# xrsrke/pipegoose

Measured on AMD Instinct MI355X. Metric: tokens/sec, higher is better.
Workload: dtype bf16; 1 GPU; model=bloom-560m, global_batch=8, seq_len=2048, parallelism=tp1pp1dp1

## Files before the change

pipegoose_amd/ops/csrc/attention.hip:

```cpp
#include <torch/extension.h>
#include <ATen/cuda/CUDAContext.h>

#include "common.h"

namespace {

using bf16 = __hip_bfloat16;
using frag_ab = __attribute__((ext_vector_type(8))) __bf16;
using frag_cd = __attribute__((ext_vector_type(4))) float;

__device__ __forceinline__ frag_cd MFMA_16x16x32(frag_ab a, frag_ab b, frag_cd c) {
    return __builtin_amdgcn_mfma_f32_16x16x32_bf16(a, b, c, 0, 0, 0);
}

constexpr int BLOCK_M = 64;
constexpr int BLOCK_N = 64;
constexpr int NWAVES = 4;
constexpr int PAD = 8;
constexpr float NEG_INF = -1e30f;


template <int D, int MT, int WAVES = NWAVES>
__global__ __launch_bounds__(WAVES * WAVE_SIZE)
void attn_fwd_kernel(const bf16* __restrict__ q, const bf16* __restrict__ k,
// ... 137 lines not shown
#pragma unroll
                for (int r = 0; r < 4; ++r) accO[mt][s][r] *= rescale[r];
            }

#pragma unroll
            for (int ns = 0; ns < 4; ++ns) {
#pragma unroll
                for (int r = 0; r < 4; ++r) {
                    float pv = __expf(s_tile[ns][r] - m_run[mt][r]);
                    s_tile[ns][r] = pv;
                    p_lds[wave][(mt * 16 + 4 * lgrp + r) * VSTRIDE + ns * 16 + lcol] =
                        (bf16)pv;
                }
            }
#pragma unroll
            for (int r = 0; r < 4; ++r) {
                float ls = s_tile[0][r] + s_tile[1][r] + s_tile[2][r] + s_tile[3][r];
#pragma unroll
                for (int off = 1; off < 16; off <<= 1) {
                    ls += __shfl_xor(ls, off, WAVE_SIZE);
                }
                l_run[mt][r] += ls;
            }
        }
        __builtin_amdgcn_s_waitcnt(0);

#pragma unroll
        for (int mt = 0; mt < MT; ++mt) {
#pragma unroll
            for (int kc = 0; kc < 2; ++kc) {
                frag_ab aP = *reinterpret_cast<const frag_ab*>(
                    &p_lds[wave][(mt * 16 + lcol) * VSTRIDE + kc * 32 + 8 * lgrp]);
                __builtin_amdgcn_s_setprio(1);
#pragma unroll
                for (int ds = 0; ds < DSUB; ++ds) {
                    frag_ab bV = *reinterpret_cast<const frag_ab*>(
                        &vt_lds[(ds * 16 + lcol) * VSTRIDE + kc * 32 + 8 * lgrp]);
                    accO[mt][ds] = MFMA_16x16x32(aP, bV, accO[mt][ds]);
                }
                __builtin_amdgcn_s_setprio(0);
            }
        }
    }

#pragma unroll
    for (int mt = 0; mt < MT; ++mt) {
#pragma unroll
        for (int r = 0; r < 4; ++r) {
            const int iq = qrow0 + mt * 16 + 4 * lgrp + r;
            const float inv_l = 1.0f / l_run[mt][r];
            bf16* orow = op + (int64_t)iq * os;
#pragma unroll
            for (int ds = 0; ds < DSUB; ++ds) {
                orow[ds * 16 + lcol] = (bf16)(accO[mt][ds][r] * inv_l);
            }
            if (lcol == 0) {
                lse[bh_off + iq] = m_run[mt][r] + __logf(l_run[mt][r]);
            }
        }
    }
}

__global__ void mfma_probe_kernel(const bf16* __restrict__ A,
                                  const bf16* __restrict__ Bt,
                                  float* __restrict__ C) {
    const int lane = threadIdx.x;
    const int lgrp = lane >> 4, lcol = lane & 15;
    frag_ab a = *reinterpret_cast<const frag_ab*>(A + lcol * 32 + 8 * lgrp);
    frag_ab b = *reinterpret_cast<const frag_ab*>(Bt + lcol * 32 + 8 * lgrp);
    frag_cd c = MFMA_16x16x32(a, b, frag_cd{0.f, 0.f, 0.f, 0.f});
#pragma unroll
    for (int r = 0; r < 4; ++r) {
        C[(4 * lgrp + r) * 16 + lcol] = c[r];
    }
}

}

__device__ __forceinline__ float u2f(unsigned u) { return __uint_as_float(u); }

namespace {

using f32x16 = __attribute__((ext_vector_type(16))) float;
using bf16x4 = __attribute__((ext_vector_type(4))) __bf16;
using lds_bf16x4_p = __attribute__((address_space(3))) bf16x4*;

__device__ __forceinline__ f32x16 MFMA_32x32x16(frag_ab a, frag_ab b, f32x16 c) {
    return __builtin_amdgcn_mfma_f32_32x32x16_bf16(a, b, c, 0, 0, 0);
}

__device__ __forceinline__ int swz128(int row, int elem_col) {
    return row * 128 + ((((elem_col) << 1) ^ ((row & 15) << 4)) >> 1);
}

__device__ __forceinline__ int swz64(int row, int elem_col) {
    return row * 64 + ((((elem_col) << 1) ^ ((row & 7) << 4)) >> 1);
}

template <int RS>
__device__ __forceinline__ int swz_rm(int row, int elem_col) {
    return RS == 64 ? swz64(row, elem_col) : swz128(row, elem_col);
}

template <int D> __device__ __forceinline__ int bwd_rm(int row, int col) {
    return D == 64 ? row * 72 + col : swz128(row, col);
}
template <int D> __device__ __forceinline__ int bwd_tr(int row, int col) {
    return D == 64 ? row * 40 + col : swz64(row, col);
}

template <int D>
__device__ __forceinline__ void pkt_rc(int p, int& row, int& col) {
    constexpr int DLOG = (D / 16 == 8) ? 3 : 2;
    const int rw = (p >> 1) & 3;
    const int dd = (p >> 3) & (D / 16 - 1);
    row = (p >> (3 + DLOG)) * 4 + rw;
    col = dd * 16 + (p & 1) * 8;
}

template <int D, int WAVES>
__global__ __launch_bounds__(WAVES * WAVE_SIZE)
void attn_fwd_v2_kernel(const bf16* __restrict__ q, const bf16* __restrict__ k,
                        const bf16* __restrict__ v,
                        const float* __restrict__ slopes, float scale,
                        bf16* __restrict__ o, float* __restrict__ lse,
                        int B, int H, int S, int kv_off, int kv_group,
                        int64_t qb, int64_t qh, int64_t qs,
                        int64_t kb, int64_t kh, int64_t ks,
                        int64_t vb, int64_t vh, int64_t vs,
                        int64_t ob, int64_t oh, int64_t os) {
    constexpr int KVB = 64;
    constexpr int NT = WAVES * WAVE_SIZE;
    constexpr int ROWS = WAVES * 32;
    constexpr int DCH = D / 16;
    constexpr int DSUB = D / 32;
    constexpr int NPK = KVB * (D / 8);
    constexpr int NPV = KVB * (D / 8);
    constexpr int KPL = (NPK + NT - 1) / NT;
    constexpr int VPL = (NPV + NT - 1) / NT;
    constexpr int VST = (D / 16) * 64;

    __shared__ __attribute__((aligned(16))) bf16 k_lds[2][KVB * 128];
    __shared__ __attribute__((aligned(16))) bf16 vs_lds[2][KVB * D];

    int qblock = blockIdx.x, h = blockIdx.y, b = blockIdx.z;
    {
        const int ngrp = gridDim.y * gridDim.z;
        if ((ngrp & 7) == 0) {
            const int flat = blockIdx.x +
                gridDim.x * (blockIdx.y + gridDim.y * blockIdx.z);
            qblock = flat / ngrp;
            const int g = flat % ngrp;
            h = g % gridDim.y;
            b = g / gridDim.y;
        }
    }
    const int tid = threadIdx.x;
    const int wave = tid / WAVE_SIZE;
    const int lane = tid % WAVE_SIZE;
    const int l31 = lane & 31;
    const int hi = lane >> 5;

    const int64_t bh_off = ((int64_t)b * H + h) * S;
    const int hk = h / kv_group;
    const bf16* qp = q + b * qb + h * qh;
    const bf16* kp = k + b * kb + hk * kh;
// ... 55 lines not shown
    auto stage_write = [&](int buf) {
#pragma unroll
        for (int i = 0; i < KPL; ++i) {
            const int p = tid + i * NT;
            if (p < NPK) {
                const int row = p / (D / 8);
                const int col = (p % (D / 8)) * 8;
                *reinterpret_cast<frag_ab*>(&k_lds[buf][swz128(row, col)]) =
                    kreg[i];
            }
        }
#pragma unroll
        for (int i = 0; i < VPL; ++i) {
            const int p = tid + i * NT;
            if (p < NPV) {
                int row, col;
                pkt_rc<D>(p, row, col);
                const int idx = (row >> 2) * VST + (col >> 4) * 64 +
                                (row & 3) * 16 + (col & 15);
                *reinterpret_cast<frag_ab*>(&vs_lds[buf][idx]) = vreg[i];
            }
        }
    };

    if (nkv > 0) {
        stage_load(0);
        stage_write(0);
    }
    __syncthreads();

    for (int nb = 0; nb < nkv; ++nb) {
        const int cur = nb & 1;
        const int kvrow0 = nb * KVB;
        const bool last = (nb + 1 == nkv);
        if (!last) stage_load(nb + 1);

        const bool active = full_vis || (kvrow0 + kv_off <= qr0 + 31);

        f32x16 st[2];
        frag_ab pfrag[4];
        if (active) {
#pragma unroll
            for (int ns = 0; ns < 2; ++ns) {
#pragma unroll
                for (int r = 0; r < 16; ++r) st[ns][r] = 0.f;
            }
#pragma unroll
            for (int ns = 0; ns < 2; ++ns) {
                __builtin_amdgcn_s_setprio(1);
#pragma unroll
                for (int c = 0; c < DCH; ++c) {
                    frag_ab aK = *reinterpret_cast<const frag_ab*>(
                        &k_lds[cur][swz128(ns * 32 + l31, c * 16 + 8 * hi)]);
                    st[ns] = MFMA_32x32x16(aK, bQ[c], st[ns]);
                }
                __builtin_amdgcn_s_setprio(0);
            }

            float mr[32];
#pragma unroll
            for (int ns = 0; ns < 2; ++ns) {
#pragma unroll
                for (int r = 0; r < 16; ++r) {
                    const int jk = kvrow0 + ns * 32 + (r & 3) + 8 * (r >> 2) +
                                   4 * hi + kv_off;
                    float x = st[ns][r] * scale2 + slope2 * (float)(jk - iq);
                    x = (jk <= iq) ? x : NEG_INF;
                    st[ns][r] = x;
                    mr[ns * 16 + r] = x;
                }
            }
#pragma unroll
            for (int w = 16; w > 0; w >>= 1) {
#pragma unroll
                for (int i = 0; i < w; ++i) mr[i] = fmaxf(mr[i], mr[i + w]);
            }
            float mx = mr[0];
            {
                auto sw = __builtin_amdgcn_permlane32_swap(
                    __float_as_uint(mx), __float_as_uint(mx), false, false);
                mx = fmaxf(u2f(sw[0]), u2f(sw[1]));
            }
            const float m_new = fmaxf(m_run, mx);
            const float alpha = exp2f(m_run - m_new);
            m_run = m_new;
            l_run *= alpha;
#pragma unroll
            for (int dsb = 0; dsb < DSUB; ++dsb) {
#pragma unroll
                for (int r = 0; r < 16; ++r) accO[dsb][r] *= alpha;
            }
            float sr[32];
#pragma unroll
            for (int ns = 0; ns < 2; ++ns) {
#pragma unroll
                for (int r = 0; r < 16; ++r) {
                    const float pv = exp2f(st[ns][r] - m_new);
                    st[ns][r] = pv;
                    sr[ns * 16 + r] = pv;
                }
            }
#pragma unroll
            for (int w = 16; w > 0; w >>= 1) {
#pragma unroll
                for (int i = 0; i < w; ++i) sr[i] += sr[i + w];
            }
            float ls = sr[0];
            {
                auto sw = __builtin_amdgcn_permlane32_swap(
                    __float_as_uint(ls), __float_as_uint(ls), false, false);
                ls = u2f(sw[0]) + u2f(sw[1]);
            }
            l_run += ls;

#pragma unroll
            for (int ns = 0; ns < 2; ++ns) {
#pragma unroll
                for (int hf = 0; hf < 2; ++hf) {
                    union { __bf16 h2[2]; uint32_t u; } wa, wb, wc, wd;
                    wa.h2[0] = (__bf16)st[ns][8 * hf + 0];
                    wa.h2[1] = (__bf16)st[ns][8 * hf + 1];
                    wc.h2[0] = (__bf16)st[ns][8 * hf + 2];
                    wc.h2[1] = (__bf16)st[ns][8 * hf + 3];
                    wb.h2[0] = (__bf16)st[ns][8 * hf + 4];
                    wb.h2[1] = (__bf16)st[ns][8 * hf + 5];
                    wd.h2[0] = (__bf16)st[ns][8 * hf + 6];
                    wd.h2[1] = (__bf16)st[ns][8 * hf + 7];
                    auto s1 = __builtin_amdgcn_permlane32_swap(wa.u, wb.u,
                                                              false, false);
                    auto s2 = __builtin_amdgcn_permlane32_swap(wc.u, wd.u,
                                                              false, false);
                    union { frag_ab f; uint32_t u[4]; } out;
                    out.u[0] = s1[0];
                    out.u[1] = s2[0];
                    out.u[2] = s1[1];
                    out.u[3] = s2[1];
                    pfrag[2 * ns + hf] = out.f;
                }
            }
        }

        if (!last) stage_write(cur ^ 1);

        if (active) {
            const int lq = lane >> 4;
            const int dblk_off = (lq & 1) * 64;
            const int lel = (lane & 15) * 4;
#pragma unroll
            for (int dsb = 0; dsb < DSUB; ++dsb) {
                __builtin_amdgcn_s_setprio(1);
#pragma unroll
                for (int ks2 = 0; ks2 < 4; ++ks2) {
                    const int g0 = 4 * ks2 + 2 * hi;
                    const int base = g0 * VST + (2 * dsb) * 64 + dblk_off + lel;
                    union { frag_ab f; bf16x4 h[2]; } av;
                    av.h[0] = __builtin_amdgcn_ds_read_tr16_b64_v4bf16(
                        (lds_bf16x4_p)&vs_lds[cur][base]);
                    av.h[1] = __builtin_amdgcn_ds_read_tr16_b64_v4bf16(
                        (lds_bf16x4_p)&vs_lds[cur][base + VST]);
                    accO[dsb] = MFMA_32x32x16(av.f, pfrag[ks2], accO[dsb]);
                }
                __builtin_amdgcn_s_setprio(0);
            }
        }
        __syncthreads();
    }

    const float inv_l = (l_run > 0.f) ? 1.0f / l_run : 0.f;
    bf16* orow = op + (int64_t)iq * os;
#pragma unroll
    for (int dsb = 0; dsb < DSUB; ++dsb) {
#pragma unroll
        for (int g = 0; g < 4; ++g) {
            union { __bf16 h4[4]; uint2 u; } w;
#pragma unroll
            for (int r = 0; r < 4; ++r) {
                w.h4[r] = (__bf16)(accO[dsb][4 * g + r] * inv_l);
            }
            *reinterpret_cast<uint2*>(orow + dsb * 32 + 8 * g + 4 * hi) = w.u;
        }
// ... 441 lines not shown
        : min((int64_t)S, (int64_t)qb * QROWS + QROWS - kv_off);
    for (int kv0 = 0; kv0 < kv_end; kv0 += KVR) {
        __syncthreads();
        {
            constexpr int PACKETS = (KVR / 2) * (D / 8);
            for (int p = tid; p < PACKETS; p += NT) {
                const int row = (p / (D / 8)) * 2;
                const int col = (p % (D / 8)) * 8;
                frag_ab pk0 = *reinterpret_cast<const frag_ab*>(
                    kp + (int64_t)(kv0 + row) * ks2 + col);
                frag_ab pk1 = *reinterpret_cast<const frag_ab*>(
                    kp + (int64_t)(kv0 + row + 1) * ks2 + col);
                frag_ab pv0 = *reinterpret_cast<const frag_ab*>(
                    vp + (int64_t)(kv0 + row) * vs2 + col);
                frag_ab pv1 = *reinterpret_cast<const frag_ab*>(
                    vp + (int64_t)(kv0 + row + 1) * vs2 + col);
                *reinterpret_cast<frag_ab*>(&k_lds[bwd_rm<D>(row, col)]) = pk0;
                *reinterpret_cast<frag_ab*>(&k_lds[bwd_rm<D>(row + 1, col)]) = pk1;
                *reinterpret_cast<frag_ab*>(&v_lds[bwd_rm<D>(row, col)]) = pv0;
                *reinterpret_cast<frag_ab*>(&v_lds[bwd_rm<D>(row + 1, col)]) = pv1;
#pragma unroll
                for (int j = 0; j < 8; ++j) {
                    union { __bf16 h[2]; uint32_t u; } a;
                    a.h[0] = pk0[j]; a.h[1] = pk1[j];
                    *reinterpret_cast<uint32_t*>(&kt_lds[bwd_tr<D>(col + j, row)]) = a.u;
                }
            }
        }
        __syncthreads();

#pragma unroll
        for (int ns = 0; ns < KVR / 16; ++ns) {
            frag_cd sacc = frag_cd{0.f, 0.f, 0.f, 0.f};
            frag_cd dpacc = frag_cd{0.f, 0.f, 0.f, 0.f};
#pragma unroll
            for (int c = 0; c < DCH; ++c) {
                frag_ab bK = *reinterpret_cast<const frag_ab*>(
                    &k_lds[bwd_rm<D>(ns * 16 + lcol, c * 32 + 8 * lgrp)]);
                sacc = MFMA_16x16x32(aQ[c], bK, sacc);
                frag_ab bV = *reinterpret_cast<const frag_ab*>(
                    &v_lds[bwd_rm<D>(ns * 16 + lcol, c * 32 + 8 * lgrp)]);
                dpacc = MFMA_16x16x32(aDO[c], bV, dpacc);
            }
#pragma unroll
            for (int r = 0; r < 4; ++r) {
                const int iq = qrow0 + 4 * lgrp + r;
                const int jk = kv0 + ns * 16 + lcol + kv_off;
                float z = sacc[r] * scale2 + slope2 * (float)(jk - iq);
                float p = (jk <= iq) ? exp2f(z - lse_r[r]) : 0.f;
                float ds = p * (dpacc[r] - delta_r[r]) * scale;
                ds_lds[wave][bwd_tr<D>(4 * lgrp + r, ns * 16 + lcol)] = (bf16)ds;
            }
        }
        __builtin_amdgcn_s_waitcnt(0);

#pragma unroll
        for (int kc = 0; kc < KVR / 32; ++kc) {
            frag_ab aDS = *reinterpret_cast<const frag_ab*>(
                &ds_lds[wave][bwd_tr<D>(lcol, kc * 32 + 8 * lgrp)]);
#pragma unroll
            for (int ds = 0; ds < DSUB; ++ds) {
                frag_ab bKT = *reinterpret_cast<const frag_ab*>(
                    &kt_lds[bwd_tr<D>(ds * 16 + lcol, kc * 32 + 8 * lgrp)]);
                accDQ[ds] = MFMA_16x16x32(aDS, bKT, accDQ[ds]);
            }
        }
    }

#pragma unroll
    for (int r = 0; r < 4; ++r) {
        const int iq = qrow0 + 4 * lgrp + r;
        bf16* dqrow = dq + b * wb + h * wh + (int64_t)iq * ws;
#pragma unroll
        for (int ds = 0; ds < DSUB; ++ds) {
            dqrow[ds * 16 + lcol] = (bf16)accDQ[ds][r];
        }
    }
}

}

namespace {

template <int D>
__device__ __forceinline__ int sub_idx(int row, int elem_col) {
    constexpr int DBLK = D / 16;
    const int g = row >> 2;
    const int dblk = (elem_col >> 4) ^ (g & (DBLK - 1));
    return g * (DBLK * 64) + dblk * 64 + (row & 3) * 16 + (elem_col & 15);
}

template <int D>
__device__ __forceinline__ int sub_tile_base(int g, int dblk_log) {
    constexpr int DBLK = D / 16;
    return g * (DBLK * 64) + (dblk_log ^ (g & (DBLK - 1))) * 64;
}

template <int D, int WAVES>
__global__ __launch_bounds__(WAVES * WAVE_SIZE)
void attn_bwd_dq_v2_kernel(const bf16* __restrict__ dout,
                           const bf16* __restrict__ q, const bf16* __restrict__ k,
                           const bf16* __restrict__ v,
                           const float* __restrict__ lse,
                           const float* __restrict__ delta,
                           const float* __restrict__ slopes, float scale,
                           bf16* __restrict__ dq,
                           int B, int H, int S, int kv_off, int kv_group,
                           int64_t gb, int64_t gh, int64_t gs,
                           int64_t qb2, int64_t qh2, int64_t qs2,
                           int64_t kb2, int64_t kh2, int64_t ks2,
                           int64_t vb2, int64_t vh2, int64_t vs2,
                           int64_t wb, int64_t wh, int64_t ws) {
    constexpr int KVB = 64;
    constexpr int NT = WAVES * WAVE_SIZE;
    constexpr int ROWS = WAVES * 32;
    constexpr int DCH = D / 16;
    constexpr int DSUB = D / 32;
    constexpr int VST = (D / 16) * 64;
    constexpr int NPK = KVB * (D / 8);
    constexpr int KPL = (NPK + NT - 1) / NT;
    constexpr int NP = (KVB / 2) * (D / 8);
    constexpr int PPL = (NP + NT - 1) / NT;

    __shared__ __attribute__((aligned(16))) bf16 ks_lds[2][KVB * D];
    __shared__ __attribute__((aligned(16))) bf16 v_lds[2][KVB * 128];

    const int qblock = blockIdx.x;
    const int h = blockIdx.y;
    const int b = blockIdx.z;
    const int tid = threadIdx.x;
    const int wave = tid / WAVE_SIZE;
    const int lane = tid % WAVE_SIZE;
    const int l31 = lane & 31;
    const int hi = lane >> 5;
    const int lq = lane >> 4;

    const int64_t bh_off = ((int64_t)b * H + h) * S;
    const int hk = h / kv_group;
    const bf16* kp = k + b * kb2 + hk * kh2;
    const bf16* vp = v + b * vb2 + hk * vh2;
    const float LOG2E = 1.4426950408889634f;
    const float scale2 = scale * LOG2E;
    const float slope2 = slopes[h] * LOG2E;

    const int qr0 = qblock * ROWS + wave * 32;
    const int iq = qr0 + l31;

    frag_ab bQ[DCH], bDO[DCH];
    {
        const bf16* qrow = q + b * qb2 + h * qh2 + (int64_t)iq * qs2;
        const bf16* dorow = dout + b * gb + h * gh + (int64_t)iq * gs;
#pragma unroll
        for (int c = 0; c < DCH; ++c) {
            bQ[c] = *reinterpret_cast<const frag_ab*>(qrow + c * 16 + 8 * hi);
            bDO[c] = *reinterpret_cast<const frag_ab*>(dorow + c * 16 + 8 * hi);
        }
    }
    const float lse2 = lse[bh_off + iq] * LOG2E;
    const float dlt = delta[bh_off + iq];

    f32x16 accDQ[DSUB];
#pragma unroll
    for (int dsb = 0; dsb < DSUB; ++dsb) {
#pragma unroll
        for (int r = 0; r < 16; ++r) accDQ[dsb][r] = 0.f;
    }

    const bool full_vis = (kv_off <= -S);
    const int kv_end = full_vis ? S
        : min(S, qblock * ROWS + ROWS - kv_off);
    const int nkv = max(0, (kv_end + KVB - 1) / KVB);

    frag_ab kreg[KPL], vreg[PPL][2];
    auto stage_load = [&](int nb) {
        const int kvrow0 = nb * KVB;
#pragma unroll
        for (int i = 0; i < KPL; ++i) {
            const int p = tid + i * NT;
            if (p < NPK) {
                int row, col;
                pkt_rc<D>(p, row, col);
                kreg[i] = *reinterpret_cast<const frag_ab*>(
                    kp + (int64_t)(kvrow0 + row) * ks2 + col);
            }
        }
#pragma unroll
        for (int i = 0; i < PPL; ++i) {
            const int p = tid + i * NT;
            if (p < NP) {
                const int row = (p / (D / 8)) * 2;
                const int col = (p % (D / 8)) * 8;
                vreg[i][0] = *reinterpret_cast<const frag_ab*>(
                    vp + (int64_t)(kvrow0 + row) * vs2 + col);
                vreg[i][1] = *reinterpret_cast<const frag_ab*>(
                    vp + (int64_t)(kvrow0 + row + 1) * vs2 + col);
            }
        }
    };
    auto stage_write = [&](int buf) {
#pragma unroll
        for (int i = 0; i < KPL; ++i) {
            const int p = tid + i * NT;
            if (p < NPK) {
                int row, col;
                pkt_rc<D>(p, row, col);
                *reinterpret_cast<frag_ab*>(
                    &ks_lds[buf][sub_idx<D>(row, col)]) = kreg[i];
            }
        }
#pragma unroll
        for (int i = 0; i < PPL; ++i) {
            const int p = tid + i * NT;
            if (p < NP) {
                const int row = (p / (D / 8)) * 2;
                const int col = (p % (D / 8)) * 8;
#pragma unroll
                for (int rr = 0; rr < 2; ++rr) {
                    *reinterpret_cast<frag_ab*>(
                        &v_lds[buf][swz128(row + rr, col)]) = vreg[i][rr];
                }
            }
        }
    };

    constexpr bool EARLY_LOAD = true;
    if (nkv > 0) {
        stage_load(0);
        stage_write(0);
    }
    __syncthreads();

    for (int nb = 0; nb < nkv; ++nb) {
        const int cur = nb & 1;
        const int kvrow0 = nb * KVB;
        const bool last = (nb + 1 == nkv);
        if (EARLY_LOAD && !last) stage_load(nb + 1);

        const bool active = full_vis || (kvrow0 + kv_off <= qr0 + 31);
        if (active) {
            auto ns_body = [&](int ns) {
                frag_ab dsfrag[2];
                f32x16 st, dp;
#pragma unroll
                for (int r = 0; r < 16; ++r) { st[r] = 0.f; dp[r] = 0.f; }
                __builtin_amdgcn_s_setprio(1);
#pragma unroll
                for (int c = 0; c < DCH; ++c) {
                    frag_ab aK = *reinterpret_cast<const frag_ab*>(
                        &ks_lds[cur][sub_idx<D>(ns * 32 + l31, c * 16 + 8 * hi)]);
                    st = MFMA_32x32x16(aK, bQ[c], st);
                    frag_ab aV = *reinterpret_cast<const frag_ab*>(
                        &v_lds[cur][swz128(ns * 32 + l31, c * 16 + 8 * hi)]);
                    dp = MFMA_32x32x16(aV, bDO[c], dp);
                }
                __builtin_amdgcn_s_setprio(0);
#pragma unroll
                for (int r = 0; r < 16; ++r) {
                    const int jk = kvrow0 + ns * 32 + (r & 3) + 8 * (r >> 2) +
                                   4 * hi + kv_off;
                    const float z2 = st[r] * scale2 +
                                     slope2 * (float)(jk - iq);
                    const float p = (jk <= iq) ? exp2f(z2 - lse2) : 0.f;
                    st[r] = p * (dp[r] - dlt) * scale;
                }
#pragma unroll
                for (int hf = 0; hf < 2; ++hf) {
                    union { __bf16 h2[2]; uint32_t u; } wa, wb2, wc, wd;
                    wa.h2[0] = (__bf16)st[8 * hf + 0];
                    wa.h2[1] = (__bf16)st[8 * hf + 1];
                    wc.h2[0] = (__bf16)st[8 * hf + 2];
                    wc.h2[1] = (__bf16)st[8 * hf + 3];
                    wb2.h2[0] = (__bf16)st[8 * hf + 4];
                    wb2.h2[1] = (__bf16)st[8 * hf + 5];
                    wd.h2[0] = (__bf16)st[8 * hf + 6];
                    wd.h2[1] = (__bf16)st[8 * hf + 7];
                    auto s1 = __builtin_amdgcn_permlane32_swap(wa.u, wb2.u,
                                                              false, false);
                    auto s2 = __builtin_amdgcn_permlane32_swap(wc.u, wd.u,
                                                              false, false);
                    union { frag_ab f; uint32_t u[4]; } out;
                    out.u[0] = s1[0];
                    out.u[1] = s2[0];
                    out.u[2] = s1[1];
                    out.u[3] = s2[1];
                    dsfrag[hf] = out.f;
                }
#pragma unroll
                for (int dsb = 0; dsb < DSUB; ++dsb) {
                    __builtin_amdgcn_s_setprio(1);
#pragma unroll
                    for (int ksq = 0; ksq < 2; ++ksq) {
                        const int g0 = 8 * ns + 4 * ksq + 2 * hi;
                        const int dblk = 2 * dsb + (lq & 1);
                        union { frag_ab f; bf16x4 h[2]; } akt;
                        akt.h[0] = __builtin_amdgcn_ds_read_tr16_b64_v4bf16(
                            (lds_bf16x4_p)&ks_lds[cur][
                                sub_tile_base<D>(g0, dblk) + (lane & 15) * 4]);
                        akt.h[1] = __builtin_amdgcn_ds_read_tr16_b64_v4bf16(
                            (lds_bf16x4_p)&ks_lds[cur][
                                sub_tile_base<D>(g0 + 1, dblk) + (lane & 15) * 4]);
                        accDQ[dsb] = MFMA_32x32x16(akt.f, dsfrag[ksq],
                                                   accDQ[dsb]);
                    }
                    __builtin_amdgcn_s_setprio(0);
                }
            };
            if (D == 128) {
#pragma unroll 1
                for (int ns = 0; ns < 2; ++ns) ns_body(ns);
            } else {
                ns_body(0);
                ns_body(1);
            }
        }
        if (!last) {
            if (!EARLY_LOAD) stage_load(nb + 1);
            stage_write(cur ^ 1);
        }
        __syncthreads();
    }

    bf16* dqrow = dq + b * wb + h * wh + (int64_t)iq * ws;
#pragma unroll
    for (int dsb = 0; dsb < DSUB; ++dsb) {
#pragma unroll
        for (int g = 0; g < 4; ++g) {
            union { __bf16 h4[4]; uint2 u; } w;
#pragma unroll
            for (int r = 0; r < 4; ++r) w.h4[r] = (__bf16)accDQ[dsb][4 * g + r];
            *reinterpret_cast<uint2*>(dqrow + dsb * 32 + 8 * g + 4 * hi) = w.u;
        }
    }
}

template <int D, int WAVES, bool DO_DK, bool DO_DV, int DKPART = -1>
__global__ __launch_bounds__(WAVES * WAVE_SIZE)
void attn_bwd_dkdv_v2_kernel(const bf16* __restrict__ dout,
                             const bf16* __restrict__ q, const bf16* __restrict__ k,
                             const bf16* __restrict__ v,
                             const float* __restrict__ lse,
                             const float* __restrict__ delta,
                             const float* __restrict__ slopes, float scale,
                             bf16* __restrict__ dk, bf16* __restrict__ dv,
                             int B, int H, int S, int kv_off, int kv_group,
                             int64_t gb, int64_t gh, int64_t gs,
                             int64_t qb2, int64_t qh2, int64_t qs2,
                             int64_t kb2, int64_t kh2, int64_t ks2,
                             int64_t vb2, int64_t vh2, int64_t vs2,
                             int64_t wb, int64_t wh, int64_t ws) {
    constexpr int QT = 64;
    constexpr int NT = WAVES * WAVE_SIZE;
    constexpr int ROWS = WAVES * 32;
    constexpr int DCH = D / 16;
    constexpr int DSUB = D / 32;
    constexpr int NP = QT * (D / 8);
    constexpr int PPL = (NP + NT - 1) / NT;

    __shared__ __attribute__((aligned(16))) bf16 qs_lds[2][QT * D];
    __shared__ __attribute__((aligned(16))) bf16 dos_lds[2][QT * D];
    __shared__ float lse_lds[2][QT];
    __shared__ float dlt_lds[2][QT];

    const int nb = blockIdx.x;
    const int h = blockIdx.y;
    const int b = blockIdx.z;
    const int tid = threadIdx.x;
    const int wave = tid / WAVE_SIZE;
    const int lane = tid % WAVE_SIZE;
    const int l31 = lane & 31;
    const int hi = lane >> 5;
    const int lq = lane >> 4;

    const int kv0w = nb * ROWS + wave * 32;
    const int n_glob = kv0w + l31;
    const float LOG2E = 1.4426950408889634f;
    const float scale2 = scale * LOG2E;

    constexpr int DK0 = (DKPART < 0) ? 0 : DKPART * (DSUB / 2);
    constexpr int NDSB = (DKPART < 0) ? DSUB : DSUB / 2;
    frag_ab bK[DCH], bV[DO_DK ? DCH : 1];
    {
        const bf16* krow = k + b * kb2 + h * kh2 + (int64_t)n_glob * ks2;
        const bf16* vrow = v + b * vb2 + h * vh2 + (int64_t)n_glob * vs2;
#pragma unroll
        for (int c = 0; c < DCH; ++c) {
            bK[c] = *reinterpret_cast<const frag_ab*>(krow + c * 16 + 8 * hi);
            if (DO_DK)
                bV[c] = *reinterpret_cast<const frag_ab*>(vrow + c * 16 + 8 * hi);
        }
    }
    f32x16 accDK[DO_DK ? NDSB : 1], accDV[DO_DV ? DSUB : 1];
#pragma unroll
    for (int dsb = 0; dsb < DSUB; ++dsb) {
#pragma unroll
        for (int r = 0; r < 16; ++r) {
            if (DO_DK && dsb < NDSB) accDK[dsb][r] = 0.f;
            if (DO_DV) accDV[dsb][r] = 0.f;
        }
    }

    const bool full_vis = (kv_off <= -S);
    const int q_first = full_vis ? 0
        : max(0, (nb * ROWS + kv_off) & ~(QT - 1));

    for (int gq = 0; gq < kv_group; ++gq) {
        const int hq = h * kv_group + gq;
        const int64_t bh_off = ((int64_t)b * H + hq) * S;
        const bf16* qp = q + b * qb2 + hq * qh2;
        const bf16* dop = dout + b * gb + hq * gh;
        const float slope2 = slopes[hq] * LOG2E;

        frag_ab qreg[PPL], doreg[PPL];
        auto stage_load = [&](int q0) {
#pragma unroll
            for (int i = 0; i < PPL; ++i) {
                const int p = tid + i * NT;
                if (p < NP) {
                    int row, col;
                    pkt_rc<D>(p, row, col);
                    qreg[i] = *reinterpret_cast<const frag_ab*>(
                        qp + (int64_t)(q0 + row) * qs2 + col);
                    doreg[i] = *reinterpret_cast<const frag_ab*>(
                        dop + (int64_t)(q0 + row) * gs + col);
                }
            }
        };
        auto stage_write = [&](int buf, int q0) {
#pragma unroll
            for (int i = 0; i < PPL; ++i) {
                const int p = tid + i * NT;
                if (p < NP) {
                    int row, col;
                    pkt_rc<D>(p, row, col);
                    *reinterpret_cast<frag_ab*>(
                        &qs_lds[buf][sub_idx<D>(row, col)]) = qreg[i];
                    *reinterpret_cast<frag_ab*>(
                        &dos_lds[buf][sub_idx<D>(row, col)]) = doreg[i];
                }
            }
            for (int i = tid; i < QT; i += NT) {
                lse_lds[buf][i] = lse[bh_off + q0 + i] * LOG2E;
                dlt_lds[buf][i] = delta[bh_off + q0 + i];
            }
        };

        constexpr bool EARLY = !(DO_DK && !DO_DV && D == 128);
        const int n_qt = (S - q_first) / QT;
        if (n_qt > 0) {
            stage_load(q_first);
            stage_write(0, q_first);
        }
        __syncthreads();

        for (int it = 0; it < n_qt; ++it) {
            const int q0 = q_first + it * QT;
            const int cur = it & 1;
            const bool last = (it + 1 == n_qt);
            if (EARLY && !last) stage_load(q0 + QT);

            const bool active = full_vis || (q0 + QT - 1 >= kv0w + kv_off);
            if (active) {
                auto qs_body = [&](int qs2c) {
                    f32x16 st, dp;
#pragma unroll
                    for (int r = 0; r < 16; ++r) { st[r] = 0.f; dp[r] = 0.f; }
                    __builtin_amdgcn_s_setprio(1);
#pragma unroll
                    for (int c = 0; c < DCH; ++c) {
                        frag_ab aQ = *reinterpret_cast<const frag_ab*>(
                            &qs_lds[cur][sub_idx<D>(qs2c * 32 + l31,
                                                    c * 16 + 8 * hi)]);
                        st = MFMA_32x32x16(aQ, bK[c], st);
                        if (DO_DK) {
                            frag_ab aDO = *reinterpret_cast<const frag_ab*>(
                                &dos_lds[cur][sub_idx<D>(qs2c * 32 + l31,
                                                         c * 16 + 8 * hi)]);
                            dp = MFMA_32x32x16(aDO, bV[c], dp);
                        }
                    }
                    __builtin_amdgcn_s_setprio(0);
                    const int jk = n_glob + kv_off;
#pragma unroll
                    for (int r = 0; r < 16; ++r) {
                        const int q_loc = qs2c * 32 + (r & 3) + 8 * (r >> 2) +
                                          4 * hi;
                        const int iq = q0 + q_loc;
                        const float z2 = st[r] * scale2 +
                                         slope2 * (float)(jk - iq);
                        const float p = (jk <= iq)
                            ? exp2f(z2 - lse_lds[cur][q_loc]) : 0.f;
                        st[r] = p;
                        if (DO_DK)
                            dp[r] = p * (dp[r] - dlt_lds[cur][q_loc]) * scale;
                    }
                    frag_ab pfrag[2], dsfrag[2];
#pragma unroll
                    for (int hf = 0; hf < 2; ++hf) {
                        union { __bf16 h2[2]; uint32_t u; } wa, wb2, wc, wd;
                        if (!DO_DV) {
                            wa.h2[0] = (__bf16)dp[8 * hf + 0];
                            wa.h2[1] = (__bf16)dp[8 * hf + 1];
                            wc.h2[0] = (__bf16)dp[8 * hf + 2];
                            wc.h2[1] = (__bf16)dp[8 * hf + 3];
                            wb2.h2[0] = (__bf16)dp[8 * hf + 4];
                            wb2.h2[1] = (__bf16)dp[8 * hf + 5];
                            wd.h2[0] = (__bf16)dp[8 * hf + 6];
                            wd.h2[1] = (__bf16)dp[8 * hf + 7];
                            auto t1 = __builtin_amdgcn_permlane32_swap(
                                wa.u, wb2.u, false, false);
                            auto t2 = __builtin_amdgcn_permlane32_swap(
                                wc.u, wd.u, false, false);
                            union { frag_ab f; uint32_t u[4]; } o2;
                            o2.u[0] = t1[0];
                            o2.u[1] = t2[0];
                            o2.u[2] = t1[1];
                            o2.u[3] = t2[1];
                            dsfrag[hf] = o2.f;
                            continue;
                        }
                        wa.h2[0] = (__bf16)st[8 * hf + 0];
                        wa.h2[1] = (__bf16)st[8 * hf + 1];
                        wc.h2[0] = (__bf16)st[8 * hf + 2];
                        wc.h2[1] = (__bf16)st[8 * hf + 3];
                        wb2.h2[0] = (__bf16)st[8 * hf + 4];
                        wb2.h2[1] = (__bf16)st[8 * hf + 5];
                        wd.h2[0] = (__bf16)st[8 * hf + 6];
                        wd.h2[1] = (__bf16)st[8 * hf + 7];
                        auto s1 = __builtin_amdgcn_permlane32_swap(
                            wa.u, wb2.u, false, false);
                        auto s2 = __builtin_amdgcn_permlane32_swap(
                            wc.u, wd.u, false, false);
                        union { frag_ab f; uint32_t u[4]; } out;
                        out.u[0] = s1[0];
                        out.u[1] = s2[0];
                        out.u[2] = s1[1];
                        out.u[3] = s2[1];
                        pfrag[hf] = out.f;
                        if (!DO_DK) continue;

                        wa.h2[0] = (__bf16)dp[8 * hf + 0];
                        wa.h2[1] = (__bf16)dp[8 * hf + 1];
                        wc.h2[0] = (__bf16)dp[8 * hf + 2];
                        wc.h2[1] = (__bf16)dp[8 * hf + 3];
                        wb2.h2[0] = (__bf16)dp[8 * hf + 4];
                        wb2.h2[1] = (__bf16)dp[8 * hf + 5];
                        wd.h2[0] = (__bf16)dp[8 * hf + 6];
                        wd.h2[1] = (__bf16)dp[8 * hf + 7];
                        s1 = __builtin_amdgcn_permlane32_swap(
                            wa.u, wb2.u, false, false);
                        s2 = __builtin_amdgcn_permlane32_swap(
                            wc.u, wd.u, false, false);
                        out.u[0] = s1[0];
                        out.u[1] = s2[0];
                        out.u[2] = s1[1];
                        out.u[3] = s2[1];
                        dsfrag[hf] = out.f;
                    }
#pragma unroll
                    for (int dsb = 0; dsb < DSUB; ++dsb) {
                        __builtin_amdgcn_s_setprio(1);
#pragma unroll
                        for (int ksq = 0; ksq < 2; ++ksq) {
                            const int g0 = qs2c * 8 + 4 * ksq + 2 * hi;
                            const int dblk = 2 * dsb + (lq & 1);
                            if (DO_DV) {
                                union { frag_ab f; bf16x4 h[2]; } adot;
                                adot.h[0] = __builtin_amdgcn_ds_read_tr16_b64_v4bf16(
                                    (lds_bf16x4_p)&dos_lds[cur][
                                        sub_tile_base<D>(g0, dblk) + (lane & 15) * 4]);
                                adot.h[1] = __builtin_amdgcn_ds_read_tr16_b64_v4bf16(
                                    (lds_bf16x4_p)&dos_lds[cur][
                                        sub_tile_base<D>(g0 + 1, dblk) + (lane & 15) * 4]);
                                accDV[DO_DV ? dsb : 0] = MFMA_32x32x16(
                                    adot.f, pfrag[ksq], accDV[DO_DV ? dsb : 0]);
                            }
                            if (DO_DK && dsb >= DK0 && dsb < DK0 + NDSB) {
                                const int dblk_k = 2 * dsb + (lq & 1);
                                union { frag_ab f; bf16x4 h[2]; } aqt;
                                aqt.h[0] = __builtin_amdgcn_ds_read_tr16_b64_v4bf16(
                                    (lds_bf16x4_p)&qs_lds[cur][
                                        sub_tile_base<D>(g0, dblk_k) + (lane & 15) * 4]);
                                aqt.h[1] = __builtin_amdgcn_ds_read_tr16_b64_v4bf16(
                                    (lds_bf16x4_p)&qs_lds[cur][
                                        sub_tile_base<D>(g0 + 1, dblk_k) + (lane & 15) * 4]);
                                const int ai = DO_DK ? dsb - DK0 : 0;
                                accDK[ai] = MFMA_32x32x16(
                                    aqt.f, dsfrag[ksq], accDK[ai]);
                            }
                        }
                        __builtin_amdgcn_s_setprio(0);
                    }
                };
                if (D == 128) {
#pragma unroll 1
                    for (int qs2c = 0; qs2c < 2; ++qs2c) qs_body(qs2c);
                } else {
                    qs_body(0);
                    qs_body(1);
                }
            }
            if (!last) {
                if (!EARLY) stage_load(q0 + QT);
                stage_write(cur ^ 1, q0 + QT);
            }
            __syncthreads();
        }
        __syncthreads();
    }

    bf16* dkrow = dk + b * wb + h * wh + (int64_t)n_glob * ws;
    bf16* dvrow = dv + b * wb + h * wh + (int64_t)n_glob * ws;
#pragma unroll
    for (int dsb = 0; dsb < DSUB; ++dsb) {
#pragma unroll
        for (int g = 0; g < 4; ++g) {
            union { __bf16 h4[4]; uint2 u; } wk2, wv2;
#pragma unroll
            for (int r = 0; r < 4; ++r) {
                if (DO_DK && dsb >= DK0 && dsb < DK0 + NDSB)
                    wk2.h4[r] = (__bf16)accDK[dsb - DK0][4 * g + r];
                if (DO_DV) wv2.h4[r] = (__bf16)accDV[dsb][4 * g + r];
            }
            if (DO_DK && dsb >= DK0 && dsb < DK0 + NDSB)
                *reinterpret_cast<uint2*>(dkrow + dsb * 32 + 8 * g + 4 * hi) = wk2.u;
            if (DO_DV)
                *reinterpret_cast<uint2*>(dvrow + dsb * 32 + 8 * g + 4 * hi) = wv2.u;
        }
    }
}

}

void attn_bwd_into(torch::Tensor dout, torch::Tensor q,
                   torch::Tensor k, torch::Tensor v,
                   torch::Tensor o, torch::Tensor lse,
                   torch::Tensor slopes, double scale,
                   torch::Tensor dq, torch::Tensor dk, torch::Tensor dv,
                   int64_t kv_off) {
    TORCH_CHECK(dout.is_cuda() && dout.stride(3) == 1 && q.stride(3) == 1 &&
                k.stride(3) == 1 && v.stride(3) == 1 && o.stride(3) == 1,
                "attn_bwd: last dim must be contiguous");
    TORCH_CHECK(dq.stride(3) == 1 && dk.stride(3) == 1 && dv.stride(3) == 1);
    TORCH_CHECK(dk.strides() == dv.strides());
    const int B = q.size(0), H = q.size(1), S = q.size(2), D = q.size(3);
    const int Hkv = k.size(1);
    TORCH_CHECK(H % Hkv == 0);
    const int kv_group = H / Hkv;
    auto delta = torch::empty({B, H, S}, q.options().dtype(torch::kFloat));

    const int64_t rows = (int64_t)B * H * S;
    auto stream = at::cuda::getCurrentCUDAStream();

    static const int use_bwd_v2 = [] {
        const char* e = getenv("PG_ATTN_BWD_V2");
        return e ? atoi(e) : 1;
    }();
    if (use_bwd_v2 && S % 128 == 0 && (D == 64 || D == 128)) {
#define STRV(t) t.stride(0), t.stride(1), t.stride(2)
#define BWD2_ARGS(W_OUT)                                                      \
            reinterpret_cast<const bf16*>(dout.data_ptr()),                   \
            reinterpret_cast<const bf16*>(q.data_ptr()),                      \
            reinterpret_cast<const bf16*>(k.data_ptr()),                      \
            reinterpret_cast<const bf16*>(v.data_ptr()),                      \
            lse.data_ptr<float>(), delta.data_ptr<float>(),                   \
            slopes.data_ptr<float>(), (float)scale, W_OUT,                    \
            B, H, S, (int)kv_off, kv_group,                                   \
            STRV(dout), STRV(q), STRV(k), STRV(v), STRV(dq)
#define LAUNCH_DELTA(DV)                                                      \
        hipLaunchKernelGGL((attn_bwd_delta_kernel<DV>),                       \
            dim3((rows + 3) / 4), dim3(256), 0, stream,                       \
            reinterpret_cast<const bf16*>(dout.data_ptr()),                   \
            reinterpret_cast<const bf16*>(o.data_ptr()),                      \
            delta.data_ptr<float>(), rows, H, S, STRV(dout), STRV(o))
#define LAUNCH_DQ2(DV, WV)                                                    \
    do {                                                                      \
        dim3 grid_q(S / (32 * WV), H, B);                                     \
        hipLaunchKernelGGL((attn_bwd_dq_v2_kernel<DV, WV>), grid_q,           \
            dim3(WV * WAVE_SIZE), 0, stream,                                  \
            BWD2_ARGS(reinterpret_cast<bf16*>(dq.data_ptr())));               \
    } while (0)
#define LAUNCH_BWD2(DV, WV, DKV, DVV, DKP)                                         \
// ... 131 lines not shown
```

Baseline: 151,100 tokens/s.

## Peel unmasked causal tiles and use fast exp2 in attention backward kernels

Switches exp2f to the hardware __builtin_amdgcn_exp2f in the forward and backward kernels. For D=64 it adds a compile-time masked/unmasked split so tiles fully below the diagonal skip the per-element causal mask select. The ALiBi bias now uses hoisted float offsets and readfirstlane'd scalar row bases. LSE and delta are read from LDS as aligned float4 vectors, and the bf16 packing is factored into a helper using vector converts. It also forces a rolled qs loop when WAVES==8, which may change register pressure and code size.

```diff
diff --git a/pipegoose_amd/ops/csrc/attention.hip b/pipegoose_amd/ops/csrc/attention.hip
--- a/pipegoose_amd/ops/csrc/attention.hip
+++ b/pipegoose_amd/ops/csrc/attention.hip
@@ -243,6 +243,7 @@
 namespace {
 
 using f32x16 = __attribute__((ext_vector_type(16))) float;
+using f32x4 = __attribute__((ext_vector_type(4))) float;
 using bf16x4 = __attribute__((ext_vector_type(4))) __bf16;
 using lds_bf16x4_p = __attribute__((address_space(3))) bf16x4*;
 
@@ -464,7 +465,7 @@
                 mx = fmaxf(u2f(sw[0]), u2f(sw[1]));
             }
             const float m_new = fmaxf(m_run, mx);
-            const float alpha = exp2f(m_run - m_new);
+            const float alpha = __builtin_amdgcn_exp2f(m_run - m_new);
             m_run = m_new;
             l_run *= alpha;
 #pragma unroll
@@ -477,7 +478,7 @@
             for (int ns = 0; ns < 2; ++ns) {
 #pragma unroll
                 for (int r = 0; r < 16; ++r) {
-                    const float pv = exp2f(st[ns][r] - m_new);
+                    const float pv = __builtin_amdgcn_exp2f(st[ns][r] - m_new);
                     st[ns][r] = pv;
                     sr[ns * 16 + r] = pv;
                 }
@@ -1085,6 +1086,35 @@
 
 namespace {
 
+template <int D> constexpr bool peel_unmasked = (D == 64);
+
+__device__ __forceinline__ float mul2_add(float a, float b, float c, float d) {
+#pragma clang fp contract(off)
+    return a * b + c * d;
+}
+
+__device__ __forceinline__ uint32_t pack_bf16x2(float lo, float hi) {
+    using f32x2 = __attribute__((ext_vector_type(2))) float;
+    using bf16x2 = __attribute__((ext_vector_type(2))) __bf16;
+    const f32x2 f = {lo, hi};
+    return __builtin_bit_cast(uint32_t, __builtin_convertvector(f, bf16x2));
+}
+
+__device__ __forceinline__ frag_ab c_to_bfrag(const f32x16& x, int hf) {
+    const uint32_t wa = pack_bf16x2(x[8 * hf + 0], x[8 * hf + 1]);
+    const uint32_t wc = pack_bf16x2(x[8 * hf + 2], x[8 * hf + 3]);
+    const uint32_t wb = pack_bf16x2(x[8 * hf + 4], x[8 * hf + 5]);
+    const uint32_t wd = pack_bf16x2(x[8 * hf + 6], x[8 * hf + 7]);
+    auto s1 = __builtin_amdgcn_permlane32_swap(wa, wb, false, false);
+    auto s2 = __builtin_amdgcn_permlane32_swap(wc, wd, false, false);
+    union { frag_ab f; uint32_t u[4]; } out;
+    out.u[0] = s1[0];
+    out.u[1] = s2[0];
+    out.u[2] = s1[1];
+    out.u[3] = s2[1];
+    return out.f;
+}
+
 template <int D>
 __device__ __forceinline__ int sub_idx(int row, int elem_col) {
     constexpr int DBLK = D / 16;
@@ -1119,6 +1149,7 @@
     constexpr int ROWS = WAVES * 32;
     constexpr int DCH = D / 16;
     constexpr int DSUB = D / 32;
+    constexpr bool PEEL = peel_unmasked<D>;
     constexpr int VST = (D / 16) * 64;
     constexpr int NPK = KVB * (D / 8);
     constexpr int KPL = (NPK + NT - 1) / NT;
@@ -1148,6 +1179,7 @@
 
     const int qr0 = qblock * ROWS + wave * 32;
     const int iq = qr0 + l31;
+    const int qr0_u = __builtin_amdgcn_readfirstlane(qr0);
 
     frag_ab bQ[DCH], bDO[DCH];
     {
@@ -1239,9 +1271,10 @@
         const bool last = (nb + 1 == nkv);
         if (EARLY_LOAD && !last) stage_load(nb + 1);
 
-        const bool active = full_vis || (kvrow0 + kv_off <= qr0 + 31);
+        const bool active = full_vis || (kvrow0 + kv_off <= qr0_u + 31);
         if (active) {
-            auto ns_body = [&](int ns) {
+            auto ns_body = [&](int ns, auto masked_t) {
+                constexpr bool MASKED = decltype(masked_t)::value;
                 frag_ab dsfrag[2];
                 f32x16 st, dp;
 #pragma unroll
@@ -1257,37 +1290,20 @@
                     dp = MFMA_32x32x16(aV, bDO[c], dp);
                 }
                 __builtin_amdgcn_s_setprio(0);
+                const int dj = kvrow0 + ns * 32 + 4 * hi + kv_off - iq;
+                const float fdj = (float)dj;
+                const bool all_live = !PEEL && full_vis;
 #pragma unroll
                 for (int r = 0; r < 16; ++r) {
-                    const int jk = kvrow0 + ns * 32 + (r & 3) + 8 * (r >> 2) +
-                                   4 * hi + kv_off;
-                    const float z2 = st[r] * scale2 +
-                                     slope2 * (float)(jk - iq);
-                    const float p = (jk <= iq) ? exp2f(z2 - lse2) : 0.f;
+                    const int roff = (r & 3) + 8 * (r >> 2);
+                    const float z2 = fmaf(slope2, fdj + (float)roff,
+                                          st[r] * scale2);
+                    float p = __builtin_amdgcn_exp2f(z2 - lse2);
+                    if (MASKED) p = (all_live || dj + roff <= 0) ? p : 0.f;
                     st[r] = p * (dp[r] - dlt) * scale;
                 }
 #pragma unroll
-                for (int hf = 0; hf < 2; ++hf) {
-                    union { __bf16 h2[2]; uint32_t u; } wa, wb2, wc, wd;
-                    wa.h2[0] = (__bf16)st[8 * hf + 0];
-                    wa.h2[1] = (__bf16)st[8 * hf + 1];
-                    wc.h2[0] = (__bf16)st[8 * hf + 2];
-                    wc.h2[1] = (__bf16)st[8 * hf + 3];
-                    wb2.h2[0] = (__bf16)st[8 * hf + 4];
-                    wb2.h2[1] = (__bf16)st[8 * hf + 5];
-                    wd.h2[0] = (__bf16)st[8 * hf + 6];
-                    wd.h2[1] = (__bf16)st[8 * hf + 7];
-                    auto s1 = __builtin_amdgcn_permlane32_swap(wa.u, wb2.u,
-                                                              false, false);
-                    auto s2 = __builtin_amdgcn_permlane32_swap(wc.u, wd.u,
-                                                              false, false);
-                    union { frag_ab f; uint32_t u[4]; } out;
-                    out.u[0] = s1[0];
-                    out.u[1] = s2[0];
-                    out.u[2] = s1[1];
-                    out.u[3] = s2[1];
-                    dsfrag[hf] = out.f;
-                }
+                for (int hf = 0; hf < 2; ++hf) dsfrag[hf] = c_to_bfrag(st, hf);
 #pragma unroll
                 for (int dsb = 0; dsb < DSUB; ++dsb) {
                     __builtin_amdgcn_s_setprio(1);
@@ -1308,12 +1324,19 @@
                     __builtin_amdgcn_s_setprio(0);
                 }
             };
+            auto ns_run = [&](int ns) {
+                if (PEEL &&
+                    (full_vis || kvrow0 + ns * 32 + 31 + kv_off <= qr0_u))
+                    ns_body(ns, std::false_type{});
+                else
+                    ns_body(ns, std::true_type{});
+            };
             if (D == 128) {
 #pragma unroll 1
-                for (int ns = 0; ns < 2; ++ns) ns_body(ns);
+                for (int ns = 0; ns < 2; ++ns) ns_run(ns);
             } else {
-                ns_body(0);
-                ns_body(1);
+                ns_run(0);
+                ns_run(1);
             }
         }
         if (!last) {
@@ -1357,12 +1380,13 @@
     constexpr int DCH = D / 16;
     constexpr int DSUB = D / 32;
     constexpr int NP = QT * (D / 8);
+    constexpr bool PEEL = peel_unmasked<D>;
     constexpr int PPL = (NP + NT - 1) / NT;
 
     __shared__ __attribute__((aligned(16))) bf16 qs_lds[2][QT * D];
     __shared__ __attribute__((aligned(16))) bf16 dos_lds[2][QT * D];
-    __shared__ float lse_lds[2][QT];
-    __shared__ float dlt_lds[2][QT];
+    __shared__ __attribute__((aligned(16))) float lse_lds[2][QT];
+    __shared__ __attribute__((aligned(16))) float dlt_lds[2][QT];
 
     const int nb = blockIdx.x;
     const int h = blockIdx.y;
@@ -1376,6 +1400,7 @@
 
     const int kv0w = nb * ROWS + wave * 32;
     const int n_glob = kv0w + l31;
+    const int kv0w_u = __builtin_amdgcn_readfirstlane(kv0w);
     const float LOG2E = 1.4426950408889634f;
     const float scale2 = scale * LOG2E;
 
@@ -1461,9 +1486,10 @@
             const bool last = (it + 1 == n_qt);
             if (EARLY && !last) stage_load(q0 + QT);
 
-            const bool active = full_vis || (q0 + QT - 1 >= kv0w + kv_off);
+            const bool active = full_vis || (q0 + QT - 1 >= kv0w_u + kv_off);
             if (active) {
-                auto qs_body = [&](int qs2c) {
+                auto qs_body = [&](int qs2c, auto masked_t) {
+                    constexpr bool MASKED = decltype(masked_t)::value;
                     f32x16 st, dp;
 #pragma unroll
                     for (int r = 0; r < 16; ++r) { st[r] = 0.f; dp[r] = 0.f; }
@@ -1482,82 +1508,36 @@
                         }
                     }
                     __builtin_amdgcn_s_setprio(0);
-                    const int jk = n_glob + kv_off;
-#pragma unroll
-                    for (int r = 0; r < 16; ++r) {
-                        const int q_loc = qs2c * 32 + (r & 3) + 8 * (r >> 2) +
-                                          4 * hi;
-                        const int iq = q0 + q_loc;
-                        const float z2 = st[r] * scale2 +
-                                         slope2 * (float)(jk - iq);
-                        const float p = (jk <= iq)
-                            ? exp2f(z2 - lse_lds[cur][q_loc]) : 0.f;
-                        st[r] = p;
+                    const int dji = n_glob + kv_off - q0 - qs2c * 32 - 4 * hi;
+                    const float fdji = (float)dji;
+                    const bool all_live = !PEEL && full_vis;
+#pragma unroll
+                    for (int g = 0; g < 4; ++g) {
+                        const f32x4 l4 = *reinterpret_cast<const f32x4*>(
+                            &lse_lds[cur][qs2c * 32 + 8 * g + 4 * hi]);
+                        f32x4 d4 = {0.f, 0.f, 0.f, 0.f};
                         if (DO_DK)
-                            dp[r] = p * (dp[r] - dlt_lds[cur][q_loc]) * scale;
+                            d4 = *reinterpret_cast<const f32x4*>(
+                                &dlt_lds[cur][qs2c * 32 + 8 * g + 4 * hi]);
+#pragma unroll
+                        for (int e = 0; e < 4; ++e) {
+                            const int r = 4 * g + e;
+                            const int roff = e + 8 * g;
+                            const float z2 = mul2_add(
+                                st[r], scale2, slope2, fdji - (float)roff);
+                            float p = __builtin_amdgcn_exp2f(z2 - l4[e]);
+                            if (MASKED)
+                                p = (all_live || dji <= roff) ? p : 0.f;
+                            st[r] = p;
+                            if (DO_DK)
+                                dp[r] = p * (dp[r] - d4[e]) * scale;
+                        }
                     }
                     frag_ab pfrag[2], dsfrag[2];
 #pragma unroll
                     for (int hf = 0; hf < 2; ++hf) {
-                        union { __bf16 h2[2]; uint32_t u; } wa, wb2, wc, wd;
-                        if (!DO_DV) {
-                            wa.h2[0] = (__bf16)dp[8 * hf + 0];
-                            wa.h2[1] = (__bf16)dp[8 * hf + 1];
-                            wc.h2[0] = (__bf16)dp[8 * hf + 2];
-                            wc.h2[1] = (__bf16)dp[8 * hf + 3];
-                            wb2.h2[0] = (__bf16)dp[8 * hf + 4];
-                            wb2.h2[1] = (__bf16)dp[8 * hf + 5];
-                            wd.h2[0] = (__bf16)dp[8 * hf + 6];
-                            wd.h2[1] = (__bf16)dp[8 * hf + 7];
-                            auto t1 = __builtin_amdgcn_permlane32_swap(
-                                wa.u, wb2.u, false, false);
-                            auto t2 = __builtin_amdgcn_permlane32_swap(
-                                wc.u, wd.u, false, false);
-                            union { frag_ab f; uint32_t u[4]; } o2;
-                            o2.u[0] = t1[0];
-                            o2.u[1] = t2[0];
-                            o2.u[2] = t1[1];
-                            o2.u[3] = t2[1];
-                            dsfrag[hf] = o2.f;
-                            continue;
-                        }
-                        wa.h2[0] = (__bf16)st[8 * hf + 0];
-                        wa.h2[1] = (__bf16)st[8 * hf + 1];
-                        wc.h2[0] = (__bf16)st[8 * hf + 2];
-                        wc.h2[1] = (__bf16)st[8 * hf + 3];
-                        wb2.h2[0] = (__bf16)st[8 * hf + 4];
-                        wb2.h2[1] = (__bf16)st[8 * hf + 5];
-                        wd.h2[0] = (__bf16)st[8 * hf + 6];
-                        wd.h2[1] = (__bf16)st[8 * hf + 7];
-                        auto s1 = __builtin_amdgcn_permlane32_swap(
-                            wa.u, wb2.u, false, false);
-                        auto s2 = __builtin_amdgcn_permlane32_swap(
-                            wc.u, wd.u, false, false);
-                        union { frag_ab f; uint32_t u[4]; } out;
-                        out.u[0] = s1[0];
-                        out.u[1] = s2[0];
-                        out.u[2] = s1[1];
-                        out.u[3] = s2[1];
-                        pfrag[hf] = out.f;
-                        if (!DO_DK) continue;
-
-                        wa.h2[0] = (__bf16)dp[8 * hf + 0];
-                        wa.h2[1] = (__bf16)dp[8 * hf + 1];
-                        wc.h2[0] = (__bf16)dp[8 * hf + 2];
-                        wc.h2[1] = (__bf16)dp[8 * hf + 3];
-                        wb2.h2[0] = (__bf16)dp[8 * hf + 4];
-                        wb2.h2[1] = (__bf16)dp[8 * hf + 5];
-                        wd.h2[0] = (__bf16)dp[8 * hf + 6];
-                        wd.h2[1] = (__bf16)dp[8 * hf + 7];
-                        s1 = __builtin_amdgcn_permlane32_swap(
-                            wa.u, wb2.u, false, false);
-                        s2 = __builtin_amdgcn_permlane32_swap(
-                            wc.u, wd.u, false, false);
-                        out.u[0] = s1[0];
-                        out.u[1] = s2[0];
-                        out.u[2] = s1[1];
-                        out.u[3] = s2[1];
-                        dsfrag[hf] = out.f;
+                        if (DO_DV) pfrag[hf] = c_to_bfrag(st, hf);
+                        if (DO_DK) dsfrag[hf] = c_to_bfrag(dp, hf);
                     }
 #pragma unroll
                     for (int dsb = 0; dsb < DSUB; ++dsb) {
@@ -1594,12 +1574,19 @@
                         __builtin_amdgcn_s_setprio(0);
                     }
                 };
-                if (D == 128) {
+                auto qs_run = [&](int qs2c) {
+                    if (PEEL &&
+                        (full_vis || kv0w_u + 31 + kv_off <= q0 + qs2c * 32))
+                        qs_body(qs2c, std::false_type{});
+                    else
+                        qs_body(qs2c, std::true_type{});
+                };
+                if (D == 128 || WAVES == 8) {
 #pragma unroll 1
-                    for (int qs2c = 0; qs2c < 2; ++qs2c) qs_body(qs2c);
+                    for (int qs2c = 0; qs2c < 2; ++qs2c) qs_run(qs2c);
                 } else {
-                    qs_body(0);
-                    qs_body(1);
+                    qs_run(0);
+                    qs_run(1);
                 }
             }
             if (!last) {
```

New measurement: 163,700 tokens/s (median of 6 runs). 1.08x the previous value.
